# kazuotani14/iLQR

Hardware: AMD Instinct MI355X
Metric: iLQR iterations/sec (batch x T timesteps/sec), acrobot T=500 batch=4096 (higher is better)
Workload: dtype f64; 1 GPU; acrobot n=4 m=1 T=499 (500 knots), box-QP limits active, FD derivatives + backward/box-QP + 11-alpha search + accept, fixed work; batch_per_gpu=4096, global_batch=4096, T=499, parallelism=batch shards x1, one all_gather of costs

## Files before the change

ilqr_amd/csrc/backward_hex.hpp:

```cpp
#pragma once
#include "solve_tile.hpp"

namespace ilqr {

#ifndef ILQR_COMMIT_ROLLED
#define ILQR_COMMIT_ROLLED 1
#endif

constexpr int HT = 4;
#ifndef ILQR_HEX_SLOT_PAD
#define ILQR_HEX_SLOT_PAD 8
#endif
#ifndef ILQR_HEX_PAIR_PERM
#define ILQR_HEX_PAIR_PERM 1
#endif
#ifndef ILQR_HEX_CAND_T
#define ILQR_HEX_CAND_T 1
#endif
constexpr bool kHexCandT = ILQR_HEX_CAND_T != 0;

template <int NX, int NU, class real, int SLOTS_>
struct HexRing {
  static constexpr int US = Rec<NX, NU>::SIZE;
  static constexpr int PAIRS = (Rec<NX, NU>::SIZE + NU + 1) / 2;
  static constexpr int ROW = 2 * HT;
  static constexpr int PAD = ROW - 2 * TW;
  static constexpr int ELEMS = PAIRS * ROW + ILQR_HEX_SLOT_PAD;
  static constexpr int SLOTS = SLOTS_;
  static constexpr bool PERM = (ILQR_HEX_PAIR_PERM != 0) && NX == 4 && NU == 1;
  static constexpr int pos(int pair) { return PERM ? hex_pair_pos(pair) : pair; }
};

constexpr int kHexKnotsPerRound = 64 / HT;
constexpr int kHexSlots = 24;
constexpr int kHexLead = 7;
static_assert(kHexSlots > kHexLead + kHexKnotsPerRound - 1, "a round must not reach a slot the chain has not left");

template <class real, int NX, int NU>
struct HexPair {
  using RS = HexRing<NX, NU, real, kHexSlots>;
  alignas(16) real ring[RS::SLOTS * RS::ELEMS];
  int rounds_done;
  int consumer_at;
  int passes_started;
  unsigned long long pass_lanes;
};

template <class P>
struct HexGate {
  static constexpr bool kRing = true;
  P& sh;
  const int T, nrounds, N;
  int pass = -1, have = 0;
  int g_next = 0, slot_next = 0, slot_cur = 0;
  __device__ __forceinline__ HexGate(P& s, int T_) : sh(s), T(T_), nrounds((T_ + 1 + kHexKnotsPerRound - 1) / kHexKnotsPerRound), N(nrounds * kHexKnotsPerRound) {}
  __device__ __forceinline__ void begin_pass() {
    pass++;
    have = pass * N;
    g_next = pass * N;
    slot_next = g_next % P::RS::SLOTS;
    __hip_atomic_store(&sh.pass_lanes, __ballot(1), __ATOMIC_RELAXED, __HIP_MEMORY_SCOPE_WORKGROUP);
    __hip_atomic_store(&sh.passes_started, pass + 1, __ATOMIC_RELEASE, __HIP_MEMORY_SCOPE_WORKGROUP);
  }
  __device__ __forceinline__ int slot(int) const { return slot_cur; }
  __device__ __forceinline__ void wait(int) {
    const int G = g_next++;
    slot_cur = slot_next;
    slot_next = (slot_next + 1 == P::RS::SLOTS) ? 0 : slot_next + 1;
    __hip_atomic_store(&sh.consumer_at, G, __ATOMIC_RELAXED, __HIP_MEMORY_SCOPE_WORKGROUP);
    if (G < have) return;
    const int round = pass * nrounds + (G - pass * N) / kHexKnotsPerRound;
    while (__hip_atomic_load(&sh.rounds_done, __ATOMIC_ACQUIRE, __HIP_MEMORY_SCOPE_WORKGROUP) <= round) __builtin_amdgcn_s_sleep(1);
    have = pass * N + ((G - pass * N) / kHexKnotsPerRound + 1) * kHexKnotsPerRound;
  }
  __device__ __forceinline__ void finish() {
    __hip_atomic_store(&sh.consumer_at, 0x3fffffff, __ATOMIC_RELAXED, __HIP_MEMORY_SCOPE_WORKGROUP);
    __hip_atomic_store(&sh.passes_started, -1, __ATOMIC_RELEASE, __HIP_MEMORY_SCOPE_WORKGROUP);
  }
};

__device__ __forceinline__ int hex_first(unsigned long long bal, int t4) {
  return __builtin_ctzll(((bal >> t4) & 0x000F000F000F000Full) | 0x8000000000000000ull);
}
__device__ __forceinline__ void qp1_search_hex(QP1StateT<double>& q, int j, int t4, double step_j0, const double* __restrict__ lds_steps) {
  const double t_x1 = clamp_of(q.x + step_j0 * q.search, q.lo, q.hi);
  const double t_v1 = qp1_value(q, t_x1);
  const bool t_pass = !qp1_armijo_fails(q, t_v1, step_j0);
  const int pp = hex_first(__ballot(t_pass), t4);
  const bool success = pp < 52;
  const int jw = success ? (((pp >> 4) << 2) | (pp & 3)) : 0;
#ifdef ILQR_EXP_NO_STEP_LDS
  q.step = jw == 0 ? 1.0 : 0.6;
#else
  q.step = lds_steps[jw];
#endif
  q.x1 = clamp_of(q.x + q.step * q.search, q.lo, q.hi);
  q.v1 = qp1_value(q, q.x1);
  bool more = p_and(!success, !q.early);
  if (__builtin_expect(__ballot(more) == 0ull, 1)) return;
  {
    const bool stuck = p_and(j >= 1, t_x1 == q.x);
    const int qs = hex_first(__ballot(p_and(stuck, more)), t4);
    if (p_and(more, qs < 52)) {
      q.ls_failed = true;
      more = false;
    }
    if (__ballot(more) == 0ull) return;
  }
  for (int base = 16;; base += 16) {
    const int kn = base + j;
    const double my_step = lds_steps[kn < 104 ? kn : 103];
    const double my_x1 = qp1_trial(q, my_step);
    const double my_v1 = qp1_value(q, my_x1);
    const bool pass = !qp1_armijo_fails(q, my_v1, my_step);
    const bool stuck = p_or(my_step < kMinStep, my_x1 == q.x);
    const int qp = hex_first(__ballot(p_and(pass, more)), t4), qs = hex_first(__ballot(p_and(stuck, more)), t4);
    if (more) {
      if (qp < qs) {
        q.step = lds_steps[base + (((qp >> 4) << 2) | (qp & 3))];
        q.x1 = qp1_trial(q, q.step);
        q.v1 = qp1_value(q, q.x1);
        more = false;
      } else if (qs < 52) {
        q.ls_failed = true;
        more = false;
      }
    }
    if (__ballot(more) == 0ull) return;
  }
}

template <class RS>
__device__ __forceinline__ int hex_pos_rt(int pair) { return RS::PERM ? hex_pair_pos(pair) : pair; }

template <class real>
struct HexStep {
  typedef real pair_t __attribute__((ext_vector_type(2)));
  real F, cxx_rc, cxx_cr, fu_r, cx_r, cxu_r, cxu_c;
  pair_t tail, uw;
};

template <class M, class Gate, class RS>
__device__ __forceinline__ void backward_hex(const BatchViewT<typename M::real>& v, const M& model, const SolverParams& sp, int mode, int tile, int sub,
                                             int lane, const double* __restrict__ lds_steps, Gate& gate, const typename M::real* __restrict__ ring) {
  using real = typename M::real;
  using creal = double;
  static_assert(M::NX == 4 && M::NU == 1, "hex chain: nx = 4, nu = 1");
  using R = Rec<4, 1>;
  typedef real real2_t __attribute__((ext_vector_type(2)));
  const int r_ = lane >> 4, t_ = (lane >> 2) & 3, c_ = lane & 3, j16 = 4 * r_ + c_;
  const int t4 = 4 * t_;
  const int l = sub * HT + t_;
  const int b = tile * TW + l;
  if (b >= v.B) return;
  if (mode == 1 && v.status[b] != 0) return;
  const int T = v.T;
  double lambda = v.lambda[b], dlambda = v.dlambda[b];
  const real* __restrict__ ust = v.us + tidx(tile, 0, 0, l, T, 1);
  real* __restrict__ kt = v.kff + tidx(tile, 0, 0, l, T, 1);
  real* __restrict__ Kt = v.Kfb + tidx(tile, 0, 0, l, T, 4);
  typedef const __attribute__((address_space(3))) real lds_cd;
  typedef const __attribute__((address_space(3))) real2_t lds_cd2;
  const creal step_j0 = lds_steps[j16];
  auto mm = [](creal a, creal bb) __attribute__((always_inline)) { return __builtin_amdgcn_mfma_f64_4x4x4f64(a, bb, 0.0, 0, 0, 0); };

  auto load = [&](int t, HexStep<real>& d) __attribute__((always_inline)) {
    gate.wait(t);
    lds_cd* r = (lds_cd*)(ring + gate.slot(t) * RS::ELEMS + t_ * 2);
    auto pair = [&](int e) { return *(lds_cd2*)(r + RS::pos(e >> 1) * RS::ROW); };
    auto one = [&](int e) { return r[hex_pos_rt<RS>(e >> 1) * RS::ROW + (e & 1)]; };
    d.F = one(R::FX + r_ + 4 * c_);
    d.cxx_rc = one(R::CXX + r_ + 4 * c_);
    d.cxx_cr = one(R::CXX + c_ + 4 * r_);
    d.fu_r = one(R::FU + r_);
    d.cx_r = one(R::CX + r_);
    d.cxu_r = one(R::CXU + r_);
    d.cxu_c = one(R::CXU + c_);
    d.tail = pair(R::CU);
    d.uw = pair(RS::US);
  };

  int diverge = 0;
  bool done = false;
  double dV0 = 0, dV1 = 0, gacc = 0;
  auto one_pass = [&]() __attribute__((always_inline)) {
    gate.begin_pass();
    creal V, RVx, kprev;
    const creal lam_r = (creal)lambda;
    {
      gate.wait(T);
      lds_cd* r = (lds_cd*)(ring + gate.slot(T) * RS::ELEMS + t_ * 2);
      RVx = (creal)r[hex_pos_rt<RS>((R::CX + r_) >> 1) * RS::ROW + ((R::CX + r_) & 1)];
      V = (creal)r[hex_pos_rt<RS>((R::CXX + r_ + 4 * c_) >> 1) * RS::ROW + ((R::CXX + r_ + 4 * c_) & 1)];
    }
    kprev = (creal)kt[(unsigned)((T - 1) * TW)];
    __builtin_amdgcn_s_waitcnt(0x0F70);
    dV0 = dV1 = 0;
    diverge = 0;
    gacc = 0;
    real* __restrict__ Kt_i = Kt + (unsigned)(((T - 1) * 4 + c_) * TW);
    real* __restrict__ kt_i = kt + (unsigned)((T - 1) * TW);

    auto step = [&](int i, const HexStep<real>& raw, HexStep<real>& nxt) -> bool {
      const creal F = (creal)raw.F, Rfu = (creal)raw.fu_r;
      const creal cu = (creal)raw.tail.x, cuu = (creal)raw.tail.y, us = (creal)raw.uw.x, usw = (creal)raw.uw.y;
      const creal W = mm(V, F);
      const creal wv = mm(V, Rfu);
      const creal aQu = mm(Rfu, RVx);
      const creal aQx = mm(F, RVx);
      const creal Tm = mm(F, W);
      const creal Tt = mm(W, F);
      const creal aQuu = mm(Rfu, wv);
      const creal aQux_c = mm(Rfu, W);
      const creal aQux_r = mm(W, Rfu);
      const creal Qxx_rc = (creal)raw.cxx_rc + Tm, Qxx_cr = (creal)raw.cxx_cr + Tt;
      const creal Qx_r = (creal)raw.cx_r + aQx;
      const creal Qu = cu + aQu;
      const creal Qux_c = (creal)raw.cxu_c + aQux_c, Qux_r = (creal)raw.cxu_r + aQux_r;
      const creal Quu = cuu + aQuu, QuuF = (cuu + lam_r) + aQuu;
      const creal lo = (creal)model.u_min[0] - us, hi = (creal)model.u_max[0] - us;
      __builtin_amdgcn_sched_barrier(0);
      if (i >= 1) load(i - 1, nxt);
      __builtin_amdgcn_sched_barrier(0);
      creal x;
      int free0;
      creal minv;
      QP1StateT<creal> q1;
      qp1_begin<false>(QuuF, Qu, kprev, lo, hi, q1, false);
      qp1_search_hex(q1, j16, t4, step_j0, lds_steps);
      bool goes_on;
      bool ok = qp1_finish_ok(q1, x, free0, minv, goes_on);
      if (goes_on)
        ok = qp1_continue(
                 q1, [&](QP1StateT<creal>& qs) __attribute__((always_inline)) { qp1_search_hex(qs, j16, t4, step_j0, lds_steps); }, x, free0) >= 1;
      if (!ok) diverge = i;
      const creal k_scale = free0 ? -minv : creal(0);
      const creal K_r = k_scale * Qux_r, K_c = k_scale * Qux_c;
      creal d0 = 0, d1 = 0;
      {
        d0 += x * Qu;
        creal rq = 0;
        rq += (creal(0.5) * x) * Quu;
        d1 += rq * x;
      }
      creal T1_r, T1_c;
      {
        creal acc = 0;
        acc += K_r * Quu;
        T1_r = acc;
      }
      {
        creal acc = 0;
        acc += K_c * Quu;
        T1_c = acc;
      }
      creal Vxn_r, Vn_rc, Vn_cr;
      {
        creal t1 = 0, t2 = 0, t3 = 0;
        t1 += T1_r * x;
        t2 += K_r * Qu;
        t3 += Qux_r * x;
        Vxn_r = ((Qx_r + t1) + t2) + t3;
      }
      {
        creal u1 = 0, u2 = 0, u3 = 0;
        u1 += T1_r * K_c;
        u2 += K_r * Qux_c;
        u3 += Qux_r * K_c;
        Vn_rc = ((Qxx_rc + u1) + u2) + u3;
      }
      {
        creal u1 = 0, u2 = 0, u3 = 0;
        u1 += T1_c * K_r;
        u2 += K_c * Qux_r;
        u3 += Qux_c * K_r;
        Vn_cr = ((Qxx_cr + u1) + u2) + u3;
      }
      V = creal(0.5) * (Vn_rc + Vn_cr);
      RVx = Vxn_r;
      if (ok) {
        dV0 += (double)d0;
        dV1 += (double)d1;
        gacc += (double)(abs_of(x) * usw);
        kprev = (creal)(real)x;
        Kt_i[0] = (real)K_c;
        kt_i[0] = (real)x;
      }
      Kt_i -= 4 * TW;
      kt_i -= TW;
      return ok;
    };

    HexStep<real> A, Bd;
    int i = T - 1;
    load(i, A);
    while (true) {
      if (!step(i, A, Bd)) break;
      if (--i < 0) break;
      if (!step(i, Bd, A)) break;
      if (--i < 0) break;
    }
  };

  while (true) {
    one_pass();
    if (mode == 0) {
      done = (diverge == 0);
      break;
    }
    if (diverge != 0) {
      dlambda = raised_dlambda(dlambda, sp);
      lambda = raised_lambda(lambda, dlambda, sp);
      if (lambda > sp.lambda_max) break;
      continue;
    }
    done = true;
    break;
  }

  double acc = gacc;
  if (!done) {
    __builtin_amdgcn_fence(__ATOMIC_RELEASE, "workgroup");
    __builtin_amdgcn_s_waitcnt(0);
    acc = 0;
    for (int t0 = 0; t0 < T; t0 += 8) {
      real kv[8], uv[8];
#pragma unroll
      for (int jj = 0; jj < 8; jj++) {
        const int t = (t0 + jj < T) ? t0 + jj : T - 1;
        kv[jj] = kt[(size_t)t * TW];
        uv[jj] = ust[(size_t)t * TW];
      }
#pragma unroll
      for (int jj = 0; jj < 8; jj++) {
        const real mx = abs_of(kv[jj]) / (abs_of(uv[jj]) + 1);
        if (t0 + jj < T) acc += (double)mx;
      }
    }
  }
  const double gnorm = acc / T;
  if (j16 == 0) {
    v.dV[b] = dV0;
    v.dV[v.Bp + b] = dV1;
    v.diverge[b] = diverge;
    v.backpass_done[b] = done ? 1 : 0;
    v.gnorm[b] = gnorm;
    if (mode == 1) {
      v.lambda[b] = lambda;
      v.dlambda[b] = dlambda;
      if (!sp.fixed_work && gnorm < sp.tol_grad && lambda < kLambdaConverged) {
        v.status[b] = 1;
        v.iters[b] += 1;
      }
    }
  }
}

template <class M, class MFD, class P>
__device__ __forceinline__ void sweep_backward_hex(const BatchViewT<typename M::real>& v, const M& model, const MFD& fdm, const SolverParams& sp, int mode,
                                                   int force, int tile, P* pairs, const double* __restrict__ lds_steps, int role) {
  using RS = typename P::RS;
  const int lane = threadIdx.x & 63;
  if (threadIdx.x < 4) {
    pairs[threadIdx.x].rounds_done = 0;
    pairs[threadIdx.x].consumer_at = 0;
    pairs[threadIdx.x].passes_started = 0;
  }
  __syncthreads();
  const int T = v.T;
  P& sh = pairs[role & 3];
  if (role < 4) {
    __builtin_amdgcn_s_setprio(3);
    HexGate<P> gate(sh, T);
    backward_hex<M, decltype(gate), RS>(v, model, sp, mode, tile, role, lane, lds_steps, gate, sh.ring);
    gate.finish();
    __builtin_amdgcn_s_setprio(0);
  } else {
    const int sub = role - 4;
    const int lp = lane & (HT - 1), ks = lane >> 2;
    const int l = sub * HT + lp;
    const int nrounds = (T + 1 + kHexKnotsPerRound - 1) / kHexKnotsPerRound, N = nrounds * kHexKnotsPerRound;
    for (int pass = 0;; pass++) {
      unsigned long long lanes = ~0ull;
      if (pass > 0) {
        int started;
        while ((started = __hip_atomic_load(&sh.passes_started, __ATOMIC_ACQUIRE, __HIP_MEMORY_SCOPE_WORKGROUP)) >= 0 && started <= pass)
          __builtin_amdgcn_s_sleep(8);
        if (started < 0) break;
        lanes = __hip_atomic_load(&sh.pass_lanes, __ATOMIC_RELAXED, __HIP_MEMORY_SCOPE_WORKGROUP);
      }
      const bool mine = (lanes >> (4 * lp)) & 1ull;
      for (int r = 0; r < nrounds; r++) {
        const int j0 = r * kHexKnotsPerRound, G0 = pass * N + j0;
        while (G0 > __hip_atomic_load(&sh.consumer_at, __ATOMIC_RELAXED, __HIP_MEMORY_SCOPE_WORKGROUP) + kHexLead) __builtin_amdgcn_s_sleep(4);
        const int started = __hip_atomic_load(&sh.passes_started, __ATOMIC_RELAXED, __HIP_MEMORY_SCOPE_WORKGROUP);
        if ((started < 0) | (started > pass + 1)) break;
        const int t = T - (j0 + ks);
        if (t >= 0 && (pass == 0 || mine))
          derivatives_of_knot<M, true, MFD, RS::PAD, RS::PERM>(v, model, fdm, force, nullptr, tile, t, l, sh.ring + ((G0 + ks) % RS::SLOTS) * RS::ELEMS + lp * 2, true);
        __builtin_amdgcn_s_waitcnt(0xC07F);
        if (lane == 0) __hip_atomic_store(&sh.rounds_done, pass * nrounds + r + 1, __ATOMIC_RELEASE, __HIP_MEMORY_SCOPE_WORKGROUP);
      }
    }
  }
}

template <class M, bool CANDT = false>
__device__ __forceinline__ void commit_tile_chunks(const BatchViewT<typename M::real>& v, const M& model, const int* commit_of_lane , int tile) {
  using real = typename M::real;
  constexpr int NX = M::NX, NU = M::NU;
  static_assert(!CANDT || (NX == 4 && NU == 1 && CT == 8 && CG == 4), "grouped candidates: nx = 4, nu = 1");
  const int T = v.T;
  const real dt = (real)v.dt;
  const int ntask = v.nch * TW;
  for (int task = threadIdx.x; task < ntask; task += blockDim.x) {
    const int l = task & (TW - 1), c = task >> 4;
    const int b = tile * TW + l;
    const int ci = (b < v.B) ? commit_of_lane[l] : -1;
    if (ci < 0) continue;
    const int ta = ci * v.ntiles + tile;
    real x[NX], uq[CT][NU];
    if constexpr (CANDT) {
      typedef real real4v __attribute__((ext_vector_type(4)));
      const real4v xv = *reinterpret_cast<const real4v*>(v.cand_x + cand_g_x(ta, c, l, v.nch, NX));
      x[0] = xv.x;
      x[1] = xv.y;
      x[2] = xv.z;
      x[3] = xv.w;
      const real4v u0 = *reinterpret_cast<const real4v*>(v.cand_u + cand_g_u(ta, 2 * c, l, T));
      const real4v u1 = *reinterpret_cast<const real4v*>(v.cand_u + cand_g_u(ta, 2 * c + 1, l, T));
      uq[0][0] = u0.x;
      uq[1][0] = u0.y;
      uq[2][0] = u0.z;
      uq[3][0] = u0.w;
      uq[4][0] = u1.x;
      uq[5][0] = u1.y;
      uq[6][0] = u1.z;
      uq[7][0] = u1.w;
    } else {
#pragma unroll
    for (int i = 0; i < NX; i++) x[i] = v.cand_x[tidx(ta, c, i, l, v.nch, NX)];
#pragma unroll
    for (int q = 0; q < CT; q++) {
      const int tq = (c * CT + q < T) ? c * CT + q : T - 1;
#pragma unroll
      for (int jj = 0; jj < NU; jj++) uq[q][jj] = v.cand_u[tidx(ta, tq, jj, l, T, NU)];
    }
    }
#if ILQR_COMMIT_ROLLED
#pragma unroll 1
    for (int q = 0; q < CT; q++) {
      const int t = c * CT + q;
      if (t > T) break;
#pragma unroll
      for (int i = 0; i < NX; i++) v.xs[tidx(tile, t, i, l, T + 1, NX)] = x[i];
      if (t < T) {
#pragma unroll
        for (int jj = 0; jj < NU; jj++) v.us[tidx(tile, t, jj, l, T, NU)] = uq[0][jj];
        if (q + 1 < CT) {
          real x1[NX];
          integrate_dynamics(model, x, uq[0], dt, x1);
#pragma unroll
          for (int i = 0; i < NX; i++) x[i] = x1[i];
        }
      }
#pragma unroll
      for (int qq = 0; qq + 1 < CT; qq++)
#pragma unroll
        for (int jj = 0; jj < NU; jj++) uq[qq][jj] = uq[qq + 1][jj];
    }
#else
#pragma unroll
    for (int q = 0; q < CT; q++) {
      const int t = c * CT + q;
      if (t <= T) {
#pragma unroll
        for (int i = 0; i < NX; i++) v.xs[tidx(tile, t, i, l, T + 1, NX)] = x[i];
        if (t < T) {
#pragma unroll
          for (int jj = 0; jj < NU; jj++) v.us[tidx(tile, t, jj, l, T, NU)] = uq[q][jj];
          if (q + 1 < CT) {
            real x1[NX];
            integrate_dynamics(model, x, uq[q], dt, x1);
#pragma unroll
            for (int i = 0; i < NX; i++) x[i] = x1[i];
          }
        }
      }
    }
#endif
  }
}

template <class M, class MFD>
__global__ __launch_bounds__(512) __attribute__((amdgpu_waves_per_eu(2, 2))) void k_solve_hex(BatchViewT<typename M::real> v, M model, MFD fdm, AlphaSet alphas,
                                                                                                 SolverParams sp, int n_iters, int force,
                                                                                                 int* __restrict__ commit_idx, int commit_pending,
                                                                                                 long long* __restrict__ phase_ticks) {
  using real = typename M::real;
  using P = HexPair<real, M::NX, M::NU>;
  __shared__ P pairs[4];
  __shared__ double steps[104];
  __shared__ double lds_cost[NALPHA * TW];
  __shared__ int tile_running;
  __shared__ int simd_count[4];
  __shared__ int lds_commit[TW];
  if (threadIdx.x < 4) simd_count[threadIdx.x] = 0;
  load_step_table(steps);
  const int wave = (int)(threadIdx.x >> 6);
  int role = wave;
  {
    const int simd = hw_simd_id();
    int slot = 0;
    if ((threadIdx.x & 63) == 0) slot = atomicAdd(&simd_count[simd], 1);
    slot = __shfl(slot, 0, 64);
    __syncthreads();
    if (simd_count[0] == 2 && simd_count[1] == 2 && simd_count[2] == 2 && simd_count[3] == 2) role = simd + 4 * slot;
  }
  const int rwave = (role < 3) ? role : 3;
  const int tile = blockIdx.x;
  constexpr int kShareReals = 4 * ((2 * M::NU + M::NU * M::NX + M::NX + 3) / 4) * TW;
  static_assert(kShareReals <= (int)(sizeof(pairs[0].ring) / sizeof(real)), "a pair's ring holds a wavefront's rollout rows");
  long long t_sweep = 0, t_roll = 0, t0 = 0;
#ifdef ILQR_HEX_SECTIONS
  long long t_sweep_last = 0;
#endif
  const bool timing = (phase_ticks != nullptr) & (threadIdx.x == 0);
  const long long c_begin = timing ? clock64() : 0, w_begin = timing ? wall_clock64() : 0;
  if (commit_pending) {
    commit_tile_chunks<M>(v, model, commit_idx + tile * TW, tile);
    phase_barrier();
  }
  int it = 0;
  for (; it < n_iters; it++) {
    if (timing) t0 = wall_clock64();
    sweep_backward_hex<M, MFD, P>(v, model, fdm, sp, 1, force, tile, pairs, steps, role);
    phase_barrier();
    if (timing) {
      const long long t1 = wall_clock64();
#ifdef ILQR_HEX_SECTIONS
      t_sweep_last = t1 - t0;
#endif
      t_sweep += t1 - t0;
      t0 = t1;
    }
    rollout_tile<M, true, true, kDeepPrefetch<M>, true, true, true, 1, kHexCandT>(v, model, alphas, NALPHA, v.cost_c, 1, sp, commit_idx, tile, lds_cost, it == n_iters - 1, rwave,
                                               pairs[role & 3].ring);
#ifdef ILQR_HEX_SECTIONS
#define ILQR_HEX_MARK(n)                                   \
    if (ILQR_HEX_SECTIONS == n && timing) {                \
      const long long t1 = wall_clock64();                 \
      t_sweep = t_sweep - t_sweep_last + (t1 - t0);        \
      t0 = t1;                                             \
    }
#else
#define ILQR_HEX_MARK(n)
#endif
    ILQR_HEX_MARK(1)
    if (threadIdx.x < TW) lds_commit[threadIdx.x] = commit_idx[tile * TW + threadIdx.x];
    if (threadIdx.x == 0) tile_running = 0;
    phase_barrier();
    ILQR_HEX_MARK(2)
    commit_tile_chunks<M, kHexCandT>(v, model, lds_commit, tile);
    ILQR_HEX_MARK(3)
    phase_barrier();
    if (timing) t_roll += wall_clock64() - t0;
    if (!sp.fixed_work) {
      const int b = tile * TW + (int)threadIdx.x;
      if (threadIdx.x < TW && b < v.B && v.status[b] == 0) tile_running = 1;
      __syncthreads();
      if (!tile_running) {
        it++;
        break;
      }
    }
  }
  if (timing) {
    phase_ticks[5 * tile + 0] += t_sweep;
    phase_ticks[5 * tile + 1] += t_roll;
    phase_ticks[5 * tile + 2] += it;
    phase_ticks[5 * tile + 3] += clock64() - c_begin;
    phase_ticks[5 * tile + 4] += wall_clock64() - w_begin;
  }
}

}
```

ilqr_amd/csrc/derivatives.hpp:

```cpp
#pragma once
#include "rollout.hpp"

namespace ilqr {

template <int N, class real, class F>
__device__ __forceinline__ void fd_hessian(const real* x, F f, real* out ) {
#pragma unroll
  for (int i = 0; i < N; i++)
#pragma unroll
    for (int j = i; j < N; j++) {
      real pp[N], pm[N], mp[N], mm[N];
#pragma unroll
      for (int l = 0; l < N; l++) pp[l] = pm[l] = mp[l] = mm[l] = x[l];
      pp[i] += real(kEps);
      pp[j] += real(kEps);
      pm[i] += real(kEps);
      pm[j] -= real(kEps);
      mp[i] -= real(kEps);
      mp[j] += real(kEps);
      mm[i] -= real(kEps);
      mm[j] -= real(kEps);
      const real v = (f(pp) - f(mp) - f(pm) + f(mm)) * real(1.0 / (4 * kEps * kEps));
      out[i + N * j] = v;
      out[j + N * i] = v;
    }
}
template <int N, class real, class F>
__device__ __forceinline__ void fd_gradient(const real* x, F f, real* out) {
#pragma unroll
  for (int i = 0; i < N; i++) {
    real p[N], m[N];
#pragma unroll
    for (int l = 0; l < N; l++) p[l] = m[l] = x[l];
    p[i] += real(kEps);
    m[i] -= real(kEps);
    out[i] = (f(p) - f(m)) * real(1.0 / (2 * kEps));
  }
}

#ifndef ILQR_RING_KB
#define ILQR_RING_KB 150
#endif
template <int NX, int NU, class real, int RING_KB = ILQR_RING_KB, int PAD = 0>
struct RingSlot {
  static constexpr int US = Rec<NX, NU>::SIZE;
  static constexpr int PAIRS = (Rec<NX, NU>::SIZE + NU + 1) / 2;
  static constexpr int ROW = 2 * TW + PAD;
  static constexpr int ELEMS = PAIRS * ROW;
  static constexpr int SLOTS = ((RING_KB * 1024 / (int)sizeof(real)) / ELEMS) / 4 * 4;
};

__host__ __device__ constexpr int hex_pair_pos(int p) {
  const int q = (p < 8) ? p : p - 12;
  if (p >= 8 && (p < 12 || p >= 20)) return p;
  const int a = (q >> 2) & 1, b = (q >> 1) & 1, c = q & 1;
  return (p - q) + 4 * a + 2 * b + (a ^ c);
}
template <class M, bool RING = false, class MFD = M, int RING_PAD = 0, bool PERM = false>
__device__ __forceinline__ void derivatives_of_knot(const BatchViewT<typename M::real>& v, const M& model, const MFD& fdm, int force,
                                                    const int* __restrict__ commit_idx, int tile, int t, int l,
                                                    typename M::real* rs = nullptr, bool records = true) {
  using real = typename M::real;
  using fdr = typename MFD::real;
  using RSl = RingSlot<M::NX, M::NU, real>;
  constexpr int NX = M::NX, NU = M::NU;
  using R = Rec<NX, NU>;
  typedef real real2_t __attribute__((ext_vector_type(2)));
  const int b = tile * TW + l;
  const int T = v.T;
  if (t > T || b >= v.B) return;
  const int ci = commit_idx ? commit_idx[b] : -1;
  const bool want = records && (force || (v.status[b] == 0 && (RING || v.flg_change[b])));
  if (ci < 0 && !want) return;
  const real dt = (real)v.dt;

  real xk[NX], uk[NU];
  {
    if (ci >= 0) {
      candidate_knot(v, model, ci, tile, t, l, xk, uk);
    } else {
#pragma unroll
      for (int i = 0; i < NX; i++) xk[i] = v.xs[tidx(tile, t, i, l, T + 1, NX)];
#pragma unroll
      for (int j = 0; j < NU; j++) uk[j] = (t < T) ? v.us[tidx(tile, t, j, l, T, NU)] : real(0);
    }
    if (ci >= 0) {
#pragma unroll
      for (int i = 0; i < NX; i++) v.xs[tidx(tile, t, i, l, T + 1, NX)] = xk[i];
      if (t < T) {
#pragma unroll
        for (int j = 0; j < NU; j++) v.us[tidx(tile, t, j, l, T, NU)] = uk[j];
      }
    }
  }
  if (!want) return;

  real* D = RING ? nullptr : v.D + didx(tile, t, 0, l, T + 1, R::SIZE);
  auto put = [&](int e, fdr val_) {
    const real val = (real)val_;
    if (RING)
      rs[(PERM ? hex_pair_pos(e >> 1) : (e >> 1)) * (2 * TW + RING_PAD) + (e & 1)] = val;
    else
      D[(size_t)(e >> 1) * (2 * TW) + (e & 1)] = val;
  };
  auto put2 = [&](int e, fdr v0, fdr v1) {
    real2_t w;
    w.x = (real)v0;
    w.y = (real)v1;
    if (RING)
      *reinterpret_cast<real2_t*>(rs + (PERM ? hex_pair_pos(e >> 1) : (e >> 1)) * (2 * TW + RING_PAD)) = w;
    else
      *reinterpret_cast<real2_t*>(D + (size_t)(e >> 1) * (2 * TW)) = w;
  };
  if (RING) {
#pragma unroll
    for (int j = 0; j < NU; j++) rs[((RSl::US + j) >> 1) * (2 * TW + RING_PAD) + ((RSl::US + j) & 1)] = uk[j];
    if constexpr (NU == 1) rs[((RSl::US + 1) >> 1) * (2 * TW + RING_PAD) + ((RSl::US + 1) & 1)] = recip(abs_of(uk[0]) + real(1));
  }

  if constexpr (has_analytic_record<M>::value) {
    if (v.analytic) {
      real rec[R::SIZE];
      model.analytic_record(xk, uk, dt, t == T, rec);
#pragma unroll
      for (int e = 0; e < R::SIZE; e += 2) put2(e, (fdr)rec[e], (fdr)rec[e + 1]);
      return;
    }
  }
  fdr x[NX], u[NU];
#pragma unroll
  for (int i = 0; i < NX; i++) x[i] = (fdr)xk[i];
#pragma unroll
  for (int j = 0; j < NU; j++) u[j] = (fdr)uk[j];
  const fdr dtf = (fdr)dt;
  const fdr inv2eps = fdr(1.0 / (2 * kEps));
  if (t < T) {
#pragma unroll
    for (int i = 0; i < NX; i++) {
      fdr p[NX], m[NX], fp[NX], fm[NX];
#pragma unroll
      for (int q = 0; q < NX; q++) p[q] = m[q] = x[q];
      p[i] += fdr(kEps);
      m[i] -= fdr(kEps);
      integrate_dynamics(fdm, p, u, dtf, fp);
      integrate_dynamics(fdm, m, u, dtf, fm);
#pragma unroll
      for (int r = 0; r < NX; r += 2)
        put2(R::FX + r + NX * i, (fp[r] - fm[r]) * inv2eps, (fp[r + 1] - fm[r + 1]) * inv2eps);
    }
#pragma unroll
    for (int i = 0; i < NU; i++) {
      fdr p[NU], m[NU], fp[NX], fm[NX];
#pragma unroll
      for (int q = 0; q < NU; q++) p[q] = m[q] = u[q];
      p[i] += fdr(kEps);
      m[i] -= fdr(kEps);
      integrate_dynamics(fdm, x, p, dtf, fp);
      integrate_dynamics(fdm, x, m, dtf, fm);
#pragma unroll
      for (int r = 0; r < NX; r += 2)
        put2(R::FU + r + NX * i, (fp[r] - fm[r]) * inv2eps, (fp[r + 1] - fm[r + 1]) * inv2eps);
    }
    fdr g[NX > NU ? NX : NU];
    fd_gradient<NX>(x, [&](const fdr* xx) { return fdm.cost(xx, u); }, g);
#pragma unroll
    for (int i = 0; i < NX; i += 2) put2(R::CX + i, g[i], g[i + 1]);
    fd_gradient<NU>(u, [&](const fdr* uu) { return fdm.cost(x, uu); }, g);
#pragma unroll
    for (int i = 0; i < NU; i++) put(R::CU + i, g[i]);
    fdr H[NX * NX];
    fd_hessian<NX>(x, [&](const fdr* xx) { return fdm.cost(xx, u); }, H);
#pragma unroll
    for (int e = 0; e < NX * NX; e += 2) put2(R::CXX + e, H[e], H[e + 1]);
  } else {
#pragma unroll
    for (int e = 0; e < NX * NX + NX * NU; e += 2) put2(R::FX + e, fdr(0), fdr(0));
    fdr g[NX];
    fd_gradient<NX>(x, [&](const fdr* xx) { return fdm.final_cost(xx); }, g);
#pragma unroll
    for (int i = 0; i < NX; i += 2) put2(R::CX + i, g[i], g[i + 1]);
#pragma unroll
    for (int i = 0; i < NU; i++) put(R::CU + i, fdr(0));
    fdr H[NX * NX];
    fd_hessian<NX>(x, [&](const fdr* xx) { return fdm.final_cost(xx); }, H);
#pragma unroll
    for (int e = 0; e < NX * NX; e += 2) put2(R::CXX + e, H[e], H[e + 1]);
  }
  {
    fdr H[NU * NU];
    fd_hessian<NU>(u, [&](const fdr* uu) { return fdm.cost(x, uu); }, H);
#pragma unroll
    for (int e = 0; e < NU * NU; e++) put(R::CUU + e, H[e]);
  }
#pragma unroll
  for (int i = 0; i < NX; i++)
#pragma unroll
    for (int j = 0; j < NU; j++) {
      fdr px[NX], mx[NX], pu[NU], mu[NU];
#pragma unroll
      for (int q = 0; q < NX; q++) px[q] = mx[q] = x[q];
#pragma unroll
      for (int q = 0; q < NU; q++) pu[q] = mu[q] = u[q];
      px[i] += fdr(kEps);
      mx[i] -= fdr(kEps);
      pu[j] += fdr(kEps);
      mu[j] -= fdr(kEps);
      fdr val;
      if (t < T)
        val = (fdm.cost(px, pu) - fdm.cost(mx, pu) - fdm.cost(px, mu) + fdm.cost(mx, mu)) * fdr(1.0 / (4 * (kEps * kEps)));
      else
        val = (fdm.final_cost(px) - fdm.final_cost(mx) - fdm.final_cost(px) + fdm.final_cost(mx)) * fdr(1.0 / (4 * (kEps * kEps)));
      put(R::CXU + i + NX * j, val);
    }
}

template <class M, class MFD = M>
__global__ __launch_bounds__(256) void k_derivatives(BatchViewT<typename M::real> v, M model, MFD fdm, int force, const int* __restrict__ commit_idx) {
  const int l = threadIdx.x & (TW - 1);
  const int t = blockIdx.x * 16 + (threadIdx.x >> 4);
  if (blockIdx.x == 0 && blockIdx.y == 0 && threadIdx.x == 0) *v.n_running = 0;
  derivatives_of_knot<M, false, MFD>(v, model, fdm, force, commit_idx, (int)blockIdx.y, t, l);
}

}
```

ilqr_amd/csrc/models.hpp:

```cpp
#pragma once
#include <type_traits>
#include <utility>

#include "boxqp.hpp"
#include "common.hpp"

namespace ilqr {

__device__ __forceinline__ int cvt_i32_saturating(double v) {
  int r;
  asm("v_cvt_i32_f64 %0, %1" : "=v"(r) : "v"(v));
  return r;
}
__device__ __forceinline__ double vreg_const(double c) {
  asm("" : "+v"(c));
  return c;
}
struct TrigConsts {
  double two_over_pi, pio2_1, pio2_2, pio2_3, s5, c5;
};
__device__ __forceinline__ TrigConsts trig_consts() {
  TrigConsts k;
  k.two_over_pi = vreg_const(6.36619772367581382433e-01);
  k.pio2_1 = vreg_const(1.57079632679489655800e+00);
  k.pio2_2 = vreg_const(6.12323399573676603587e-17);
  k.pio2_3 = vreg_const(-1.49738490485916983294e-33);
  k.s5 = vreg_const(-2.50507602534068634195e-08);
  k.c5 = vreg_const(2.08757232129817482790e-09);
  return k;
}
__device__ __forceinline__ void sincos_shared(double x, double& s_out, double& c_out, const TrigConsts& k) {
#pragma clang fp contract(on)
  const double j = __builtin_rint(x * k.two_over_pi);
  double r = __builtin_fma(-j, k.pio2_1, x);
  r = __builtin_fma(-j, k.pio2_2, r);
  r = __builtin_fma(-j, k.pio2_3, r);
  const unsigned q = (unsigned)cvt_i32_saturating(j);
  r = __hiloint2double(__double2hiint(r) ^ (int)(((q + 1u) << 30) & 0x80000000u), __double2loint(r));
  const double z = r * r;
  const double ps = 8.33333333332248946124e-03 +
                    z * (-1.98412698298579493134e-04 +
                         z * (2.75573137070700676789e-06 + z * (k.s5 + z * 1.58969099521155010221e-10)));
  const double sr = r + (z * r) * (-1.66666666666666324348e-01 + z * ps);
  const double pc = z * (4.16666666666666019037e-02 +
                         z * (-1.38888888888741095749e-03 +
                              z * (2.48015872894767294178e-05 +
                                   z * (-2.75573143513906633035e-07 +
                                        z * (k.c5 + z * -1.13596475577881948265e-11)))));
  const double hz = 0.5 * z;
  const double w = 1.0 - hz;
  double cr = w + (((1.0 - w) - hz) + z * pc);
  cr = __hiloint2double(__double2hiint(cr) ^ (int)((q << 30) & 0x80000000u), __double2loint(cr));
  s_out = (q & 1u) ? cr : sr;
  c_out = (q & 1u) ? sr : cr;
}

__device__ __forceinline__ void sincos_shared(double x, double& s_out, double& c_out) { sincos_shared(x, s_out, c_out, trig_consts()); }
struct NoTrigConsts {};
__device__ __forceinline__ void sincos_shared(float x, float& s_out, float& c_out, const NoTrigConsts&);

__device__ __forceinline__ void sincos_shared(float x, float& s_out, float& c_out) {
#pragma clang fp contract(on)
  const double xd = (double)x;
  const double j = __builtin_rint(xd * 6.36619772367581382433e-01);
  const unsigned q = (unsigned)cvt_i32_saturating(j);
  const float r = __uint_as_float(__float_as_uint((float)__builtin_fma(-j, 1.57079632679489655800e+00, xd)) ^ (((q + 1u) << 30) & 0x80000000u));
  const float z = r * r;
  const float sr = r + (z * r) * (-1.6666654611e-1f + z * (8.3321608736e-3f + z * -1.9515295891e-4f));
  const float cr = __uint_as_float(__float_as_uint((1.0f - 0.5f * z) + (z * z) * (4.166664568298827e-2f + z * (-1.388731625493765e-3f + z * 2.443315711809948e-5f))) ^
                                  ((q << 30) & 0x80000000u));
  s_out = (q & 1u) ? cr : sr;
  c_out = (q & 1u) ? sr : cr;
}

__device__ __forceinline__ void sincos_shared(float x, float& s_out, float& c_out, const NoTrigConsts&) { sincos_shared(x, s_out, c_out); }
template <class real> struct TrigConstsOf { using type = NoTrigConsts; static __device__ __forceinline__ type get() { return type(); } };
template <> struct TrigConstsOf<double> { using type = TrigConsts; static __device__ __forceinline__ type get() { return trig_consts(); } };

template <class real_>
struct AcrobotModelT {
  using real = real_;
  static constexpr int NX = 4;
  static constexpr int NU = 1;
  real goal[4];
  real u_min[1], u_max[1];

  using trig_consts_t = typename TrigConstsOf<real>::type;
  __device__ __forceinline__ void dynamics(const real* x, const real* u, real* dx) const { dynamics_k(x, u, dx, TrigConstsOf<real>::get()); }
  __device__ __forceinline__ void dynamics_k(const real* x, const real* u, real* dx, const trig_consts_t& tk) const {
#pragma clang fp contract(on)
    const real I1 = 1, I2 = 1, l1 = 1, l2 = 1, m1 = 1, m2 = 1, g = real(9.81);
    const real lc1 = real(0.5) * l1, lc2 = real(0.5) * l2;
    const real q0 = x[0], q1 = x[1], qd0 = x[2], qd1 = x[3];
    real s1, c1, s2, c2;
    sincos_shared(q0, s1, c1, tk);
    sincos_shared(q1, s2, c2, tk);
    const real s12 = s1 * c2 + c1 * s2;
    const real H00 = I1 + I2 + m2 * l1 * l1 + 2 * m2 * l1 * lc2 * c2;
    const real H01 = I2 + m2 * l1 * lc2 * c2;
    const real H10 = H01;
    const real H11 = I2;
    const real C00 = -2 * m2 * l1 * lc2 * s2 * qd1;
    const real C01 = -m2 * l2 * lc2 * s2 * qd1;
    const real C10 = m2 * l1 * lc2 * s2 * qd0;
    const real G0 = m1 * g * lc1 * s1 + m2 * g * (l1 * s1 + lc2 * s12);
    const real G1 = m2 * g * lc2 * s12;
    const real r0 = (real(0.0) - (C00 * qd0 + C01 * qd1)) - G0;
    const real r1 = (u[0] - (C10 * qd0)) - G1;
    const real invdet = recip(H00 * H11 - H10 * H01);
    dx[0] = qd0;
    dx[1] = qd1;
    dx[2] = (H11 * invdet) * r0 + (-H01 * invdet) * r1;
    dx[3] = (-H10 * invdet) * r0 + (H00 * invdet) * r1;
  }
  __device__ __forceinline__ void analytic_record(const real* x, const real* u, real dt, bool last, real* rec) const {
    using R = Rec<4, 1>;
#pragma unroll
    for (int e = 0; e < R::SIZE; e++) rec[e] = real(0);
    rec[R::CUU] = 2 * real(0.1) * real(0.1);
    if (last) {
#pragma unroll
      for (int i = 0; i < 4; i++) {
        rec[R::CX + i] = -real(2.0) * real(400.0) * (goal[i] - x[i]);
        rec[R::CXX + i + 4 * i] = real(2.0) * real(400.0);
      }
      return;
    }
    const real g = real(9.81), b = real(0.5);
    const real qd0 = x[2], qd1 = x[3];
    real s1, c1, s2, c2;
    sincos_shared(x[0], s1, c1);
    sincos_shared(x[1], s2, c2);
    const real s12 = s1 * c2 + c1 * s2, c12 = c1 * c2 - s1 * s2;
    const real H00 = real(3.0) + 2 * b * c2, H01 = real(1.0) + b * c2, H11 = real(1.0);
    const real Cq0 = -2 * b * s2 * qd1 * qd0 - b * s2 * qd1 * qd1, Cq1 = b * s2 * qd0 * qd0;
    const real G0 = g * (real(1.5) * s1 + real(0.5) * s12), G1 = real(0.5) * g * s12;
    const real r0 = -Cq0 - G0, r1 = u[0] - Cq1 - G1;
    const real invdet = real(1.0) / (H00 * H11 - H01 * H01);
    const real a0 = invdet * (H11 * r0 - H01 * r1), a1 = invdet * (-H01 * r0 + H00 * r1);
    real dr[5][2];
    dr[0][0] = -g * (real(1.5) * c1 + real(0.5) * c12);
    dr[0][1] = -real(0.5) * g * c12;
    {
      const real dC0 = -2 * b * c2 * qd1 * qd0 - b * c2 * qd1 * qd1, dC1 = b * c2 * qd0 * qd0;
      const real dG = real(0.5) * g * c12;
      const real dH00 = -2 * b * s2, dH01 = -b * s2;
      dr[1][0] = -dC0 - dG - (dH00 * a0 + dH01 * a1);
      dr[1][1] = -dC1 - dG - (dH01 * a0);
    }
    dr[2][0] = 2 * b * s2 * qd1;
    dr[2][1] = -2 * b * s2 * qd0;
    dr[3][0] = 2 * b * s2 * qd0 + 2 * b * s2 * qd1;
    dr[3][1] = real(0.0);
    dr[4][0] = real(0.0);
    dr[4][1] = real(1.0);
    real dq[5][2];
#pragma unroll
    for (int z = 0; z < 5; z++) {
      dq[z][0] = invdet * (H11 * dr[z][0] - H01 * dr[z][1]);
      dq[z][1] = invdet * (-H01 * dr[z][0] + H00 * dr[z][1]);
    }
#pragma unroll
    for (int c = 0; c < 4; c++) {
      rec[R::FX + c + 4 * c] = real(1.0);
      rec[R::FX + 2 + 4 * c] += dt * dq[c][0];
      rec[R::FX + 3 + 4 * c] += dt * dq[c][1];
    }
    rec[R::FX + 0 + 4 * 2] += dt;
    rec[R::FX + 1 + 4 * 3] += dt;
    rec[R::FU + 2] = dt * dq[4][0];
    rec[R::FU + 3] = dt * dq[4][1];
    rec[R::CU] = 2 * real(0.1) * real(0.1) * u[0];
  }

  __device__ __forceinline__ real cost(const real* x, const real* u) const {
#pragma clang fp contract(on)
    (void)x;
    const real Kr = real(0.1);
    return Kr * Kr * (u[0] * u[0]);
  }
  __device__ __forceinline__ real final_cost(const real* x) const {
#pragma clang fp contract(on)
    const real q0 = goal[0] - x[0], q1 = goal[1] - x[1];
    const real qd0 = goal[2] - x[2], qd1 = goal[3] - x[3];
    const real Ks = real(20.0), Kd = real(20.0);
    return Ks * Ks * (q0 * q0 + q1 * q1) + Kd * Kd * (qd0 * qd0 + qd1 * qd1);
  }
};

template <class real_>
struct DoubleIntegratorModelT {
  using real = real_;
  static constexpr int NX = 4;
  static constexpr int NU = 2;
  real goal[4];
  real u_min[2], u_max[2];

  __device__ __forceinline__ void dynamics(const real* x, const real* u, real* dx) const {
#pragma clang fp contract(on)
    const real mass = real(1.0);
    dx[0] = x[2];
    dx[1] = x[3];
    dx[2] = u[0] / mass;
    dx[3] = u[1] / mass;
  }
  __device__ __forceinline__ real quad(const real* x, real scale) const {
#pragma clang fp contract(on)
    const real hx[4] = {1, 1, real(0.2), real(0.2)};
    real d[4], r[4];
#pragma unroll
    for (int i = 0; i < 4; i++) {
      d[i] = goal[i] - x[i];
      r[i] = scale * (hx[i] * d[i]);
    }
    return (r[0] * d[0] + r[2] * d[2]) + (r[1] * d[1] + r[3] * d[3]);
  }
  __device__ __forceinline__ void analytic_record(const real* x, const real* u, real dt, bool last, real* rec) const {
    using R = Rec<4, 2>;
    const real hx[4] = {1, 1, real(0.2), real(0.2)};
#pragma unroll
    for (int e = 0; e < R::SIZE; e++) rec[e] = real(0);
    const real scale = last ? real(10.0) : real(1.0);
#pragma unroll
    for (int i = 0; i < 4; i++) {
      rec[R::CX + i] = -real(2.0) * scale * hx[i] * (goal[i] - x[i]);
      rec[R::CXX + i + 4 * i] = real(2.0) * scale * hx[i];
    }
    rec[R::CUU + 0] = real(2.0);
    rec[R::CUU + 3] = real(2.0);
    if (last) return;
#pragma unroll
    for (int c = 0; c < 4; c++) rec[R::FX + c + 4 * c] = real(1.0);
    rec[R::FX + 0 + 4 * 2] = dt;
    rec[R::FX + 1 + 4 * 3] = dt;
    rec[R::FU + 2 + 4 * 0] = dt;
    rec[R::FU + 3 + 4 * 1] = dt;
    rec[R::CU + 0] = real(2.0) * u[0];
    rec[R::CU + 1] = real(2.0) * u[1];
  }
  __device__ __forceinline__ real cost(const real* x, const real* u) const {
#pragma clang fp contract(on)
    return quad(x, real(1.0)) + (u[0] * u[0] + u[1] * u[1]);
  }
  __device__ __forceinline__ real final_cost(const real* x) const { return quad(x, real(10.0)); }
};

template <class M, class = void>
struct WithTrigConsts : M {
  __device__ __forceinline__ explicit WithTrigConsts(const M& m) : M(m) {}
};
template <class M>
struct WithTrigConsts<M, std::void_t<typename M::trig_consts_t>> : M {
  using real = typename M::real;
  typename M::trig_consts_t tk;
  __device__ __forceinline__ explicit WithTrigConsts(const M& m) : M(m), tk(TrigConstsOf<real>::get()) {}
  __device__ __forceinline__ void dynamics(const real* x, const real* u, real* dx) const { M::dynamics_k(x, u, dx, tk); }
};

template <class M>
__device__ __forceinline__ void integrate_dynamics(const M& m, const typename M::real* x, const typename M::real* u, typename M::real dt,
                                                   typename M::real* x1) {
#pragma clang fp contract(on)
  typename M::real dx[M::NX];
  m.dynamics(x, u, dx);
#pragma unroll
  for (int i = 0; i < M::NX; i++) x1[i] = x[i] + dx[i] * dt;
}

using AcrobotModel = AcrobotModelT<double>;
using DoubleIntegratorModel = DoubleIntegratorModelT<double>;

template <class M, class = void>
struct has_analytic_record : std::false_type {};
template <class M>
struct has_analytic_record<M, std::void_t<decltype(std::declval<const M&>().analytic_record((const typename M::real*)nullptr, (const typename M::real*)nullptr,
                                                                                            typename M::real(0), false, (typename M::real*)nullptr))>> : std::true_type {};

template <class M, class = void>
struct has_trajectory_params : std::false_type {};
template <class M>
struct has_trajectory_params<M, std::void_t<decltype(M::NTP), decltype(std::declval<M&>().set_trajectory_params((const double*)nullptr))>> : std::true_type {};
template <class M, bool = has_trajectory_params<M>::value>
struct trajectory_params_count : std::integral_constant<int, 0> {};
template <class M>
struct trajectory_params_count<M, true> : std::integral_constant<int, M::NTP> {};

}

#ifdef ILQR_USER_MODEL_HEADER
namespace ilqr {
#include ILQR_USER_MODEL_HEADER
static_assert(UserModelT<double>::NX >= 1 && UserModelT<double>::NX <= MAXN && UserModelT<double>::NU >= 1 && UserModelT<double>::NU <= kMaxControls,
              "user device models: 1 <= NX <= 32, 1 <= NU <= 32");
constexpr bool kUserQuad = UserModelT<double>::NX == 4 && (UserModelT<double>::NU == 1 || UserModelT<double>::NU == 2);
constexpr bool kUserSmall = !kUserQuad && UserModelT<double>::NX % 2 == 0 && UserModelT<double>::NX <= 8 && UserModelT<double>::NU <= 4;
constexpr bool kUserTiled = kUserQuad || kUserSmall;
constexpr bool kUserGeneric = !kUserQuad;
constexpr int kUserNTP = trajectory_params_count<UserModelT<double>>::value;
static_assert(kUserNTP == trajectory_params_count<UserModelT<float>>::value, "UserModelT<float> and UserModelT<double> take the same per-trajectory parameters");
static_assert(!has_trajectory_params<UserModelT<double>>::value || (kUserNTP >= 1 && kUserNTP <= 64), "user device models: 1 <= NTP <= 64");
}
#define ILQR_HAVE_USER_MODEL 1
#else
namespace ilqr { constexpr bool kUserTiled = false, kUserSmall = false; constexpr int kUserNTP = 0; }
#endif
```

Before: 4.318 billion trajectory-timesteps/s.

## Compact ring records for state-free running cost to deepen producer lead

For the acrobot, whose running cost does not depend on state, ring slots now hold only the dynamics Jacobians, the control cost terms and the control value. The zero state-cost terms are read from a single zero cell, and the terminal gradient and Hessian get a separate term buffer. Because each slot is smaller, more slots fit in the same LDS, so the derivative producers can run further ahead of the backward chain and stall less on the ring. The cost is a specialized layout that applies only to this model, plus extra template branching.

```diff
diff --git a/ilqr_amd/csrc/backward_hex.hpp b/ilqr_amd/csrc/backward_hex.hpp
--- a/ilqr_amd/csrc/backward_hex.hpp
+++ b/ilqr_amd/csrc/backward_hex.hpp
@@ -19,26 +19,48 @@
 #endif
 constexpr bool kHexCandT = ILQR_HEX_CAND_T != 0;
 
-template <int NX, int NU, class real, int SLOTS_>
+template <int NX, int NU, class real, int SLOTS_, bool COMPACT_ = false>
 struct HexRing {
+  static constexpr bool COMPACT = COMPACT_;
   static constexpr int US = Rec<NX, NU>::SIZE;
-  static constexpr int PAIRS = (Rec<NX, NU>::SIZE + NU + 1) / 2;
+  static constexpr int PAIRS = COMPACT ? CompactRec<NX, NU>::PAIRS : (Rec<NX, NU>::SIZE + NU + 1) / 2;
   static constexpr int ROW = 2 * HT;
   static constexpr int PAD = ROW - 2 * TW;
   static constexpr int ELEMS = PAIRS * ROW + ILQR_HEX_SLOT_PAD;
+  static constexpr int Z = PAIRS * ROW;
+  static_assert(!COMPACT || ILQR_HEX_SLOT_PAD >= ROW, "the compact slot keeps Z in its pad row");
+  static_assert(!COMPACT || (NX == 4 && NU == 1), "compact slots: nx = 4, nu = 1");
   static constexpr int SLOTS = SLOTS_;
   static constexpr bool PERM = (ILQR_HEX_PAIR_PERM != 0) && NX == 4 && NU == 1;
-  static constexpr int pos(int pair) { return PERM ? hex_pair_pos(pair) : pair; }
+  static constexpr int pos(int pair) { return PERM && (!COMPACT || pair < 8) ? hex_pair_pos(pair) : pair; }
 };
 
 constexpr int kHexKnotsPerRound = 64 / HT;
-constexpr int kHexSlots = 24;
-constexpr int kHexLead = 7;
-static_assert(kHexSlots > kHexLead + kHexKnotsPerRound - 1, "a round must not reach a slot the chain has not left");
-
-template <class real, int NX, int NU>
-struct HexPair {
-  using RS = HexRing<NX, NU, real, kHexSlots>;
+constexpr int kHexFullSlots = 24;
+template <int NX, int NU, class real, bool COMPACT>
+struct HexRingSize {
+  using Full = HexRing<NX, NU, real, kHexFullSlots, false>;
+  static constexpr int TERM = COMPACT ? ((NX + NX * NX) / 2) * Full::ROW : 0;
+  static constexpr int SLOTS = COMPACT ? (kHexFullSlots * Full::ELEMS - TERM) / HexRing<NX, NU, real, 1, COMPACT>::ELEMS : kHexFullSlots;
+  static constexpr int LEAD = SLOTS - kHexKnotsPerRound - 1;
+  static_assert(SLOTS > LEAD + kHexKnotsPerRound - 1 && LEAD >= 1, "a round must not reach a slot the chain has not left");
+  static_assert(SLOTS * HexRing<NX, NU, real, 1, COMPACT>::ELEMS + TERM <= kHexFullSlots * Full::ELEMS, "the pair's records fit the bytes of 24 full slots");
+};
+
+template <class real, int N>
+struct HexTerm {
+  alignas(16) real term[N];
+};
+template <class real>
+struct HexTerm<real, 0> {
+  static constexpr real* term = nullptr;
+};
+
+template <class real, int NX, int NU, bool COMPACT = false>
+struct HexPair : HexTerm<real, HexRingSize<NX, NU, real, COMPACT>::TERM> {
+  using Size = HexRingSize<NX, NU, real, COMPACT>;
+  using RS = HexRing<NX, NU, real, Size::SLOTS, COMPACT>;
+  static constexpr int LEAD = Size::LEAD;
   alignas(16) real ring[RS::SLOTS * RS::ELEMS];
   int rounds_done;
   int consumer_at;
@@ -131,7 +153,7 @@
 }
 
 template <class RS>
-__device__ __forceinline__ int hex_pos_rt(int pair) { return RS::PERM ? hex_pair_pos(pair) : pair; }
+__device__ __forceinline__ int hex_pos_rt(int pair) { return RS::pos(pair); }
 
 template <class real>
 struct HexStep {
@@ -142,7 +164,8 @@
 
 template <class M, class Gate, class RS>
 __device__ __forceinline__ void backward_hex(const BatchViewT<typename M::real>& v, const M& model, const SolverParams& sp, int mode, int tile, int sub,
-                                             int lane, const double* __restrict__ lds_steps, Gate& gate, const typename M::real* __restrict__ ring) {
+                                             int lane, const double* __restrict__ lds_steps, Gate& gate, const typename M::real* __restrict__ ring,
+                                             const typename M::real* __restrict__ term ) {
   using real = typename M::real;
   using creal = double;
   static_assert(M::NX == 4 && M::NU == 1, "hex chain: nx = 4, nu = 1");
@@ -169,6 +192,15 @@
     lds_cd* r = (lds_cd*)(ring + gate.slot(t) * RS::ELEMS + t_ * 2);
     auto pair = [&](int e) { return *(lds_cd2*)(r + RS::pos(e >> 1) * RS::ROW); };
     auto one = [&](int e) { return r[hex_pos_rt<RS>(e >> 1) * RS::ROW + (e & 1)]; };
+    if constexpr (RS::COMPACT) {
+      using C = CompactRec<4, 1>;
+      d.F = one(C::FX + r_ + 4 * c_);
+      d.fu_r = one(C::FU + r_);
+      d.cxx_rc = d.cxx_cr = d.cx_r = d.cxu_r = d.cxu_c = r[RS::Z];
+      d.tail = pair(C::CU);
+      d.uw = pair(C::US);
+      return;
+    }
     d.F = one(R::FX + r_ + 4 * c_);
     d.cxx_rc = one(R::CXX + r_ + 4 * c_);
     d.cxx_cr = one(R::CXX + c_ + 4 * r_);
@@ -189,9 +221,16 @@
     const creal lam_r = (creal)lambda;
     {
       gate.wait(T);
+      if constexpr (RS::COMPACT) {
+        using C = CompactRec<4, 1>;
+        lds_cd* r = (lds_cd*)(term + t_ * 2);
+        RVx = (creal)r[((C::TERM_CX + r_) >> 1) * RS::ROW + ((C::TERM_CX + r_) & 1)];
+        V = (creal)r[((C::TERM_CXX + r_ + 4 * c_) >> 1) * RS::ROW + ((C::TERM_CXX + r_ + 4 * c_) & 1)];
+      } else {
       lds_cd* r = (lds_cd*)(ring + gate.slot(T) * RS::ELEMS + t_ * 2);
       RVx = (creal)r[hex_pos_rt<RS>((R::CX + r_) >> 1) * RS::ROW + ((R::CX + r_) & 1)];
       V = (creal)r[hex_pos_rt<RS>((R::CXX + r_ + 4 * c_) >> 1) * RS::ROW + ((R::CXX + r_ + 4 * c_) & 1)];
+      }
     }
     kprev = (creal)kt[(unsigned)((T - 1) * TW)];
     __builtin_amdgcn_s_waitcnt(0x0F70);
@@ -372,7 +411,7 @@
   if (role < 4) {
     __builtin_amdgcn_s_setprio(3);
     HexGate<P> gate(sh, T);
-    backward_hex<M, decltype(gate), RS>(v, model, sp, mode, tile, role, lane, lds_steps, gate, sh.ring);
+    backward_hex<M, decltype(gate), RS>(v, model, sp, mode, tile, role, lane, lds_steps, gate, sh.ring, sh.term);
     gate.finish();
     __builtin_amdgcn_s_setprio(0);
   } else {
@@ -392,12 +431,17 @@
       const bool mine = (lanes >> (4 * lp)) & 1ull;
       for (int r = 0; r < nrounds; r++) {
         const int j0 = r * kHexKnotsPerRound, G0 = pass * N + j0;
-        while (G0 > __hip_atomic_load(&sh.consumer_at, __ATOMIC_RELAXED, __HIP_MEMORY_SCOPE_WORKGROUP) + kHexLead) __builtin_amdgcn_s_sleep(4);
+        while (G0 > __hip_atomic_load(&sh.consumer_at, __ATOMIC_RELAXED, __HIP_MEMORY_SCOPE_WORKGROUP) + P::LEAD) __builtin_amdgcn_s_sleep(4);
         const int started = __hip_atomic_load(&sh.passes_started, __ATOMIC_RELAXED, __HIP_MEMORY_SCOPE_WORKGROUP);
         if ((started < 0) | (started > pass + 1)) break;
         const int t = T - (j0 + ks);
-        if (t >= 0 && (pass == 0 || mine))
-          derivatives_of_knot<M, true, MFD, RS::PAD, RS::PERM>(v, model, fdm, force, nullptr, tile, t, l, sh.ring + ((G0 + ks) % RS::SLOTS) * RS::ELEMS + lp * 2, true);
+        if (t >= 0 && (pass == 0 || mine)) {
+          typename M::real* rs = sh.ring + ((G0 + ks) % RS::SLOTS) * RS::ELEMS + lp * 2;
+          if constexpr (RS::COMPACT) {
+            if (t == T) rs = sh.term + lp * 2;
+          }
+          derivatives_of_knot<M, true, MFD, RS::PAD, RS::PERM, RS::COMPACT>(v, model, fdm, force, nullptr, tile, t, l, rs, true);
+        }
         __builtin_amdgcn_s_waitcnt(0xC07F);
         if (lane == 0) __hip_atomic_store(&sh.rounds_done, pass * nrounds + r + 1, __ATOMIC_RELEASE, __HIP_MEMORY_SCOPE_WORKGROUP);
       }
@@ -498,7 +542,7 @@
                                                                                                  int* __restrict__ commit_idx, int commit_pending,
                                                                                                  long long* __restrict__ phase_ticks) {
   using real = typename M::real;
-  using P = HexPair<real, M::NX, M::NU>;
+  using P = HexPair<real, M::NX, M::NU, state_free_running_cost<M>::value>;
   __shared__ P pairs[4];
   __shared__ double steps[104];
   __shared__ double lds_cost[NALPHA * TW];
diff --git a/ilqr_amd/csrc/derivatives.hpp b/ilqr_amd/csrc/derivatives.hpp
--- a/ilqr_amd/csrc/derivatives.hpp
+++ b/ilqr_amd/csrc/derivatives.hpp
@@ -4,7 +4,7 @@
 namespace ilqr {
 
 template <int N, class real, class F>
-__device__ __forceinline__ void fd_hessian(const real* x, F f, real* out ) {
+__host__ __device__ __forceinline__ void fd_hessian(const real* x, F f, real* out ) {
 #pragma unroll
   for (int i = 0; i < N; i++)
 #pragma unroll
@@ -26,7 +26,7 @@
     }
 }
 template <int N, class real, class F>
-__device__ __forceinline__ void fd_gradient(const real* x, F f, real* out) {
+__host__ __device__ __forceinline__ void fd_gradient(const real* x, F f, real* out) {
 #pragma unroll
   for (int i = 0; i < N; i++) {
     real p[N], m[N];
@@ -56,7 +56,15 @@
   const int a = (q >> 2) & 1, b = (q >> 1) & 1, c = q & 1;
   return (p - q) + 4 * a + 2 * b + (a ^ c);
 }
-template <class M, bool RING = false, class MFD = M, int RING_PAD = 0, bool PERM = false>
+template <int NX, int NU>
+struct CompactRec {
+  static constexpr int FX = 0, FU = FX + NX * NX, CU = FU + NX * NU, CUU = CU + NU, US = CUU + NU * NU, SIZE = US + NU + 1;
+  static constexpr int PAIRS = SIZE / 2;
+  static constexpr int Z = 2 * PAIRS;
+  static constexpr int TERM_CX = 0, TERM_CXX = NX, TERM_PAIRS = (NX + NX * NX) / 2;
+  static constexpr int pos(int pair, bool perm) { return (perm && pair < 8) ? hex_pair_pos(pair) : pair; }
+};
+template <class M, bool RING = false, class MFD = M, int RING_PAD = 0, bool PERM = false, bool COMPACT = false>
 __device__ __forceinline__ void derivatives_of_knot(const BatchViewT<typename M::real>& v, const M& model, const MFD& fdm, int force,
                                                     const int* __restrict__ commit_idx, int tile, int t, int l,
                                                     typename M::real* rs = nullptr, bool records = true) {
@@ -65,6 +73,8 @@
   using RSl = RingSlot<M::NX, M::NU, real>;
   constexpr int NX = M::NX, NU = M::NU;
   using R = Rec<NX, NU>;
+  static_assert(!COMPACT || (RING && state_free_running_cost<M>::value && state_free_running_cost<MFD>::value),
+                "compact records: the ring of a model whose running cost ignores the state");
   typedef real real2_t __attribute__((ext_vector_type(2)));
   const int b = tile * TW + l;
   const int T = v.T;
@@ -95,6 +105,85 @@
   }
   if (!want) return;
 
+  if constexpr (COMPACT) {
+    using C = CompactRec<NX, NU>;
+    constexpr int ROW = 2 * TW + RING_PAD;
+    auto cput2 = [&](int row, fdr v0, fdr v1) {
+      real2_t w;
+      w.x = (real)v0;
+      w.y = (real)v1;
+      *reinterpret_cast<real2_t*>(rs + row * ROW) = w;
+    };
+    const bool exact = has_analytic_record<M>::value && v.analytic;
+    real rec[R::SIZE];
+    if constexpr (has_analytic_record<M>::value) {
+      if (exact) model.analytic_record(xk, uk, dt, t == T, rec);
+    }
+    fdr x[NX], u[NU];
+#pragma unroll
+    for (int i = 0; i < NX; i++) x[i] = (fdr)xk[i];
+#pragma unroll
+    for (int j = 0; j < NU; j++) u[j] = (fdr)uk[j];
+    const fdr dtf = (fdr)dt;
+    const fdr inv2eps = fdr(1.0 / (2 * kEps));
+    if (t == T) {
+      fdr g[NX], H[NX * NX];
+      if (exact) {
+#pragma unroll
+        for (int i = 0; i < NX; i++) g[i] = (fdr)rec[R::CX + i];
+#pragma unroll
+        for (int e = 0; e < NX * NX; e++) H[e] = (fdr)rec[R::CXX + e];
+      } else {
+        fd_gradient<NX>(x, [&](const fdr* xx) { return fdm.final_cost(xx); }, g);
+        fd_hessian<NX>(x, [&](const fdr* xx) { return fdm.final_cost(xx); }, H);
+      }
+#pragma unroll
+      for (int i = 0; i < NX; i += 2) cput2((C::TERM_CX + i) >> 1, g[i], g[i + 1]);
+#pragma unroll
+      for (int e = 0; e < NX * NX; e += 2) cput2((C::TERM_CXX + e) >> 1, H[e], H[e + 1]);
+      return;
+    }
+    rs[(C::US >> 1) * ROW] = uk[0];
+    rs[(C::US >> 1) * ROW + 1] = recip(abs_of(uk[0]) + real(1));
+    if (exact) {
+#pragma unroll
+      for (int e = 0; e < NX * NX + NX * NU; e += 2) cput2(C::pos((C::FX + e) >> 1, PERM), (fdr)rec[R::FX + e], (fdr)rec[R::FX + e + 1]);
+      cput2(C::CU >> 1, (fdr)rec[R::CU], (fdr)rec[R::CUU]);
+      rs[(C::Z >> 1) * ROW] = real(0);
+      return;
+    }
+#pragma unroll
+    for (int i = 0; i < NX; i++) {
+      fdr p[NX], m[NX], fp[NX], fm[NX];
+#pragma unroll
+      for (int q = 0; q < NX; q++) p[q] = m[q] = x[q];
+      p[i] += fdr(kEps);
+      m[i] -= fdr(kEps);
+      integrate_dynamics(fdm, p, u, dtf, fp);
+      integrate_dynamics(fdm, m, u, dtf, fm);
+#pragma unroll
+      for (int r = 0; r < NX; r += 2)
+        cput2(C::pos((C::FX + r + NX * i) >> 1, PERM), (fp[r] - fm[r]) * inv2eps, (fp[r + 1] - fm[r + 1]) * inv2eps);
+    }
+    {
+      fdr p[NU], m[NU], fp[NX], fm[NX];
+      p[0] = m[0] = u[0];
+      p[0] += fdr(kEps);
+      m[0] -= fdr(kEps);
+      integrate_dynamics(fdm, x, p, dtf, fp);
+      integrate_dynamics(fdm, x, m, dtf, fm);
+#pragma unroll
+      for (int r = 0; r < NX; r += 2)
+        cput2((C::FU + r) >> 1, (fp[r] - fm[r]) * inv2eps, (fp[r + 1] - fm[r + 1]) * inv2eps);
+    }
+    fdr g[NU], H[NU * NU];
+    fd_gradient<NU>(u, [&](const fdr* uu) { return fdm.cost(x, uu); }, g);
+    fd_hessian<NU>(u, [&](const fdr* uu) { return fdm.cost(x, uu); }, H);
+    cput2(C::CU >> 1, g[0], H[0]);
+    const fdr c = fdm.cost(x, u);
+    rs[(C::Z >> 1) * ROW] = (real)(c - c);
+    return;
+  }
   real* D = RING ? nullptr : v.D + didx(tile, t, 0, l, T + 1, R::SIZE);
   auto put = [&](int e, fdr val_) {
     const real val = (real)val_;
diff --git a/ilqr_amd/csrc/models.hpp b/ilqr_amd/csrc/models.hpp
--- a/ilqr_amd/csrc/models.hpp
+++ b/ilqr_amd/csrc/models.hpp
@@ -173,7 +173,7 @@
     rec[R::CU] = 2 * real(0.1) * real(0.1) * u[0];
   }
 
-  __device__ __forceinline__ real cost(const real* x, const real* u) const {
+  __host__ __device__ __forceinline__ real cost(const real* x, const real* u) const {
 #pragma clang fp contract(on)
     (void)x;
     const real Kr = real(0.1);
@@ -275,6 +275,11 @@
 template <class M>
 struct has_analytic_record<M, std::void_t<decltype(std::declval<const M&>().analytic_record((const typename M::real*)nullptr, (const typename M::real*)nullptr,
                                                                                             typename M::real(0), false, (typename M::real*)nullptr))>> : std::true_type {};
+
+template <class M>
+struct state_free_running_cost : std::false_type {};
+template <class real>
+struct state_free_running_cost<AcrobotModelT<real>> : std::true_type {};
 
 template <class M, class = void>
 struct has_trajectory_params : std::false_type {};
```

Result: faster. 4.383 billion trajectory-timesteps/s (median of 6 runs) (+1.5%).
